# Alandroid/img-compression-mps

Measured on AMD Instinct MI355X. Metric: Mvoxels/s compress+reconstruct, 256^3 fp32, bond chi=64; SSIM vs ref, higher is better.
Workload: dtype f32

## Files before the change

### img-compression-mps_amd/_lib.py

```python
import ctypes as C
import os

_HERE = os.path.dirname(os.path.abspath(__file__))
LIB_PATH = os.path.join(_HERE, "libndmps_hip.so")

OK, EINVAL, EHIP, ENOCONV, EWORKSPACE, ETEAM = 0, -1, -2, -3, -4, -5

i64 = C.c_int64
p_i64 = C.POINTER(C.c_int64)
p_f64 = C.POINTER(C.c_double)
p_f32 = C.POINTER(C.c_float)
p_int = C.POINTER(C.c_int)
vp = C.c_void_p

SIGNATURES = {
    "ndmps_version": (C.c_int, []),
    "ndmps_last_error": (C.c_char_p, []),
    "ndmps_device_count": (C.c_int, []),
    "ndmps_streams_create": (C.c_int, [C.c_int, C.POINTER(vp), C.POINTER(C.c_int)]),
    "ndmps_streams_destroy": (C.c_int, [C.c_int, C.POINTER(vp)]),
    "ndmps_profile_enable": (C.c_int, [C.c_int]),
    "ndmps_profile_collect": (C.c_int, [C.c_int, p_f64, p_i64, p_i64]),
    "ndmps_plan_create": (C.c_int, [C.POINTER(vp), C.c_int, p_i64, C.c_int, p_i64]),
    "ndmps_plan_create_reversed": (C.c_int, [C.POINTER(vp), C.c_int, p_i64, C.c_int, p_i64]),
# ... 86 lines not shown
    "ndmps_syevj_batched_workspace_bytes": (i64, [i64, C.c_int]),
    "ndmps_syevj_batched_f64": (C.c_int, [C.c_int, vp, i64, p_i64, vp, i64, vp, i64, vp, i64, p_int, vp]),
    "ndmps_syevj_batched_tol_f64": (C.c_int, [C.c_int, vp, i64, p_i64, vp, i64, vp, i64, C.c_double, vp, i64,
                                              p_int, vp]),
    "ndmps_syevj_batched_values_f64": (C.c_int, [C.c_int, vp, i64, p_i64, vp, i64, vp, i64, C.c_double, vp, i64,
                                                 p_int, vp]),
    "ndmps_syevj_batched_vectors_f64": (C.c_int, [C.c_int, vp, i64, p_i64, vp, i64, vp, i64, p_i64, vp, i64, vp]),
    "ndmps_syevd_topk_max_n": (i64, []),
    "ndmps_syevd_topk_max_k": (i64, []),
    "ndmps_syevd_topk_max_k_wide": (i64, []),
    "ndmps_potrf_scratch_elems": (i64, [i64]),
    "ndmps_potrf_lower_f64": (C.c_int, [vp, i64, vp, C.POINTER(C.c_int), vp]),
    "ndmps_syevd_topk_workspace_bytes": (i64, [i64, C.c_int, i64]),
    "ndmps_syevd_topk_stamps_offset": (i64, [i64, C.c_int, i64]),
    "ndmps_syevd_topk_values_f64": (C.c_int, [C.c_int, vp, i64, p_i64, vp, i64, vp, i64, i64, vp, i64, vp]),
    "ndmps_syevd_topk_vectors_f64": (C.c_int, [C.c_int, p_i64, p_i64, i64, vp, i64, p_int, vp]),
    "ndmps_syevd_topk_vectors_auto_f64": (C.c_int, [C.c_int, p_i64, i64, C.c_double, vp, vp, i64, vp, vp, i64, vp]),
    "ndmps_syevd_topk_recover_f64": (C.c_int, [C.c_int, p_i64, i64, vp, i64, p_int, vp]),
    "ndmps_syevd_topk_set_team": (C.c_int, [C.c_int]),
    "ndmps_syevd_topk_set_streamed": (C.c_int, [C.c_int]),
    "ndmps_syevd_topk_team_fallbacks": (i64, []),
    "ndmps_syevd_topk_team_slots": (C.c_int, [i64]),
    "ndmps_syevd_topk_note_team_fallback": (C.c_int, []),
    "ndmps_debug_inject_team_abort": (C.c_int, [C.c_int]),
    "ndmps_debug_lane_sums_f64": (C.c_int, [vp, vp, vp]),
    "ndmps_tt_sweep_pads_cores": (C.c_int, [C.c_int, p_i64, i64]),
    "ndmps_tt_sweep_async_ints": (i64, [C.c_int, C.c_int]),
    "ndmps_tt_sweep_async_doubles": (i64, [C.c_int, C.c_int, p_i64, i64]),
    "ndmps_tt_sweep_batched_fused_begin_f32": (C.c_int, [C.c_int, C.POINTER(vp), C.c_int, p_i64, C.c_double, i64,
                                                         C.POINTER(vp), p_i64, p_i64, vp, vp, vp, vp, vp, i64,
                                                         vp, i64, vp, vp, vp]),
    "ndmps_tt_sweep_finish": (C.c_int, [C.c_int, C.c_int, p_i64, i64, vp, vp, p_i64, p_f64, p_i64]),
    "ndmps_tt_sweep_batched_workspace_bytes": (i64, [C.c_int, C.c_int, p_i64, i64]),
    "ndmps_tt_sweep_batched_f32": (C.c_int, [C.c_int, C.POINTER(vp), C.c_int, p_i64, C.c_double, i64,
                                             C.POINTER(vp), p_i64, p_i64, p_f64, p_i64, vp, i64, vp]),
    "ndmps_tt_layout": (C.c_int, [C.c_int, p_i64, i64, p_i64, p_i64, p_i64, p_i64]),
    "ndmps_tt_sweep_f32": (C.c_int, [vp, C.c_int, p_i64, C.c_double, i64, vp, p_i64, p_i64, p_f64,
                                     p_i64, vp, i64, vp]),
    "ndmps_compress_bond_workspace_bytes": (i64, [i64, i64, i64, i64, i64]),
    "ndmps_compress_bond_f32": (C.c_int, [vp, vp, i64, i64, i64, i64, i64, C.c_double, i64, vp, vp,
                                          p_i64, p_f64, vp, i64, vp]),
    "ndmps_chain_workspace_bytes": (i64, [C.c_int, p_i64, p_i64]),
    "ndmps_chain_contract_f32": (C.c_int, [C.c_int, p_i64, p_i64, C.POINTER(vp), vp, vp, i64, vp]),
    "ndmps_overlap_workspace_bytes": (i64, [C.c_int, p_i64, p_i64, p_i64]),
    "ndmps_overlap_f32": (C.c_int, [C.c_int, p_i64, p_i64, C.POINTER(vp), p_i64, C.POINTER(vp), p_f64,
                                    vp, i64, vp]),
# ... 96 lines not shown
```

### img-compression-mps_amd/csrc/eig_sym.inc

```
constexpr int kSymTiles = 17;

struct SymShared {
  double bc[4];
  RowVec rv[512];
  double red_a[4], red_b[4];
  double part[4][64];
  double rsum[kSymTiles * 32];
  int go;
};

template <int NB>
__device__ __forceinline__ void trd_sym_body(SymShared& sh, TrdDesc& d, const TrdWork& w, const int64_t b, const int wg) {
  constexpr int NR = 2, NT = kSymTiles;
  const int n = d.n;
  const int J = n - kTail;
  const int nblk = (n + 31) / 32;
  const int nphys = (nblk + 1) / 2;
  const int blkA = wg, blkB = nblk - 1 - wg;
  const int nA = nblk - blkA;
  const int nB = blkB != blkA ? NB : 0;
  const int j_last = min(J - 1, 32 * blkB + 30);
  const int lda = w.lda;
  const int tid = threadIdx.x, lane = tid & 63, wave = tid >> 6;
  double* A = w.A + b * w.n_max * lda;
  double* Vh = w.Vh + b * w.n_max * lda;
  double* ycol = w.y + b * 2 * lda;
  double* yrow = w.yrow + b * 2 * 8 * lda;
  double* xc = w.xc + b * 2 * lda;
  TeamSync* sync = w.sync + b;
  double (&bc)[4] = sh.bc;
  RowVec (&rv)[512] = sh.rv;
  double (&red_a)[4] = sh.red_a;
  double (&red_b)[4] = sh.red_b;
  double (&part)[4][64] = sh.part;
  double (&rsum)[kSymTiles * 32] = sh.rsum;
  int& go = sh.go;

  const int p = lane & 7, q = lane >> 3;
// ... 258 lines not shown
    const int r_lo = J >> 5;
#pragma unroll
    for (int r = 0; r < NR; ++r) {
      const int i = tid + 256 * r;
      if (i >= J && i < n) {
        double s = team_load(yc + i);
        const int bm = i >> 5;
        for (int ws = 0; ws < nphys; ++ws) {
          const int ra = ws, rb = nblk - 1 - ws;
          if ((ra >= r_lo && ra < bm) || (rb != ra && rb >= r_lo && rb < bm)) s += team_load(yr + (int64_t)ws * lda + i);
        }
        yc[i] = s;
      }
    }
  }
}

__global__ void __launch_bounds__(256, 2)
trd_sym_kernel(TrdDesc* __restrict__ desc, TrdWork w, int b0) {
  int wg, team;
  if (!team_place(w, wg, team)) return;
  const int64_t b = b0 + team;
  TrdDesc& d = desc[b];
  if (d.n - kTail <= 0 || wg >= ((d.n + 31) / 32 + 1) / 2) return;
  __shared__ SymShared sh;
  switch (wg) {
    case 0: trd_sym_body<1>(sh, d, w, b, wg); break;
    case 1: trd_sym_body<2>(sh, d, w, b, wg); break;
    case 2: trd_sym_body<3>(sh, d, w, b, wg); break;
    case 3: trd_sym_body<4>(sh, d, w, b, wg); break;
    case 4: trd_sym_body<5>(sh, d, w, b, wg); break;
    case 5: trd_sym_body<6>(sh, d, w, b, wg); break;
    case 6: trd_sym_body<7>(sh, d, w, b, wg); break;
    default: trd_sym_body<8>(sh, d, w, b, wg); break;
  }
}
```

### img-compression-mps_amd/csrc/eig_tridiag.hip

```cpp
#include <math.h>
#include <stdlib.h>
#include <string.h>

#include <algorithm>
#include <atomic>
#include <map>
#include <mutex>
#include <vector>

#include "common.h"
#include "lanes.h"

namespace {
__device__ __forceinline__ double load_if(const double* p, bool ok) {
  const double v = *p;
  return ok ? v : 0.0;
}
}

namespace {

typedef double f64x4 __attribute__((ext_vector_type(4)));

constexpr int kTail = 128;
constexpr int kTailLd = 132;
constexpr int kMaxK = 128;
constexpr int kMaxN = 4096;

struct TrdDesc {
  const double* G_in;
  double* V_out;
  double* w_out;
  int n;
  int k;
  int status;
  int pad;
};

struct __attribute__((aligned(16))) TeamRec {
  double v;
  unsigned long long tag;
};

struct TeamSync {
  unsigned long long count;
  int abort;
  int pad[317];
};
// ... 3 lines not shown
  double* Vh;
  double* y;
  double* xc;
  TeamRec* yr;
  TeamRec* xr;
  TeamSync* sync;
  double* tau;
  double* d;
  double* e;
  double* lam;
  double* mu;
  double* bound;
  double* Z;
  double* lu;
  unsigned char* piv;
  double* Tw;
  int64_t t_stride;
  double* yb;
  double* xb;
  double* band;
  double* qlog;
  int64_t q_stride;
  int tail_lower;
  int xcd_team, xcd_count;
  int xcd_pair;
  double* yrow;
  double* pv;
  double* pw;
  double* ypart;
  double* spart;
  double* ucol;
  double* napart;
  int pnl_blocks_max, pnl_tiles_max;
  long long* stamps;
  int n_max, lda, kp;
};

template <int STEPS>
__device__ __forceinline__ double fast_rsqrt(double x) {
  double y = __builtin_amdgcn_rsq(x);
#pragma unroll
  for (int i = 0; i < STEPS; ++i) y = y * fma(-0.5 * x * y, y, 1.5);
  return y;
}
template <int STEPS>
__device__ __forceinline__ double fast_rcp(double x) {
// ... 37 lines not shown
  const int n = d.n, lda = w.lda;
  const double* G = d.G_in;
  double* A = w.A + (int64_t)blockIdx.y * w.n_max * lda;
  const int64_t total = (int64_t)n * lda;
  for (int64_t e = (int64_t)blockIdx.x * 256 + threadIdx.x; e < total; e += (int64_t)gridDim.x * 256) {
    const int r = (int)(e / lda), c = (int)(e % lda);
    A[e] = c < n ? 0.5 * (G[(int64_t)r * n + c] + G[(int64_t)c * n + r]) : 0.0;
  }
}

struct __attribute__((aligned(16))) RowVec {
  double vp, wp, vj, pad;
};

template <int NR, int CW>
__global__ void __launch_bounds__(256)
trd_column_kernel(const TrdDesc* __restrict__ desc, TrdWork w, int j) {
  constexpr int LPR = CW / 2;
  constexpr int RPW = 64 / LPR;
  constexpr int RPI = 4 * RPW;
  constexpr int PRE = 512 / RPI;
  const TrdDesc& d = desc[blockIdx.y];
  const int n = d.n;
  if (j >= n - kTail) return;
  const int c0 = blockIdx.x * CW;
  if (c0 >= n || c0 + CW <= j + 1) return;
  const int lda = w.lda;
  const int tid = threadIdx.x, lane = tid & 63, wave = tid >> 6;
  const int64_t b = blockIdx.y;
  double* A = w.A + b * w.n_max * lda;
  double* Vh = w.Vh + b * w.n_max * lda;
  double* ybuf = w.y + b * 2 * lda;
  extern __shared__ __attribute__((aligned(16))) double lds[];
  RowVec* rv = reinterpret_cast<RowVec*>(lds);
  __shared__ double red_a[4], red_b[4];
  __shared__ double part[4][CW];

  const int q = lane / LPR, p = lane % LPR;
  const int c = c0 + 2 * p;
  const bool col_ok = c < lda;
  const int first = j + 1 + RPW * wave + q;
  double2 a[PRE];
#pragma unroll
  for (int u = 0; u < PRE; ++u) {
    const int i = first + RPI * u;
    a[u] = (i < n && col_ok) ? *reinterpret_cast<const double2*>(A + (int64_t)i * lda + c) : make_double2(0.0, 0.0);
  }
// ... 195 lines not shown
      const int blk = min(w.xcd_team, 32), pos = member % blk;
      member += blk - 1 - 2 * pos;
    }
  } else {
    const int r = w.xcd_count - full, l2 = L - full * w.xcd_team;
    member = l2 / r;
    team = full + l2 % r;
  }
  return true;
}

template <int NR, bool TAGGED, int CW = 32>
__global__ void __launch_bounds__(256, NR <= 4 ? 2 : 1)
trd_team_kernel(TrdDesc* __restrict__ desc, TrdWork w, int b0, unsigned epoch) {
  constexpr int MR = 256 * NR;
  constexpr int LPR = CW / 4;
  constexpr int RPW = 64 / LPR;
  constexpr int RPI = 4 * RPW;
  constexpr int NT = MR / RPI;
  int member, team;
  if (!team_place(w, member, team)) return;
  TrdDesc& d = desc[b0 + team];
  const int n = d.n;
  const int J = n - kTail;
  const int c0 = member * CW;
  if (J <= 0 || c0 >= n) return;
  const int nblk = (n + CW - 1) / CW;
  const int j_last = min(J - 1, c0 + CW - 2);
  const int lda = w.lda;
  const int tid = threadIdx.x, lane = tid & 63, wave = tid >> 6;
  const int64_t b = b0 + team;
  double* A = w.A + b * w.n_max * lda;
  double* Vh = w.Vh + b * w.n_max * lda;
  double* ybuf = w.y + b * 2 * lda;
  double* xc = w.xc + b * 2 * lda;
  TeamSync* sync = w.sync + b;
  TeamRec* yr = w.yr + b * 2 * lda;
  TeamRec* xr = w.xr + b * 2 * lda;
  const unsigned long long tag_base = (unsigned long long)epoch << 32;
  extern __shared__ __attribute__((aligned(32))) double team_dyn[];
  RowVec* rv = reinterpret_cast<RowVec*>(team_dyn);
  __shared__ double red_a[4], red_b[4];
  __shared__ double part[4][CW];
  __shared__ int go;

  const int q = lane % RPW, p = lane / RPW;
  const int c = c0 + 4 * p;
// ... 294 lines not shown
    __syncthreads();
    TEAM_STAMP(6)
    if (!go) return;
  }
#ifdef NDMPS_TEAM_STAMPS
  if (tid == 0 && member == nblk - 1)
    for (int q = 0; q < 8; ++q) w.stamps[b * 16 + q] = st[q];
#endif

  if (j_last == J - 1) {
    const int u0 = J / RPI;
#pragma unroll
    for (int u = 0; u < NT; ++u) {
      const int i = row0 + RPI * u;
      if (u >= u0 && i < n) {
        if (c < lda) *reinterpret_cast<double2*>(A + (int64_t)i * lda + c) = make_double2(a[u][0], a[u][1]);
        if (c + 2 < lda) *reinterpret_cast<double2*>(A + (int64_t)i * lda + c + 2) = make_double2(a[u][2], a[u][3]);
      }
    }
  }
}

__global__ void __launch_bounds__(512) trd_tail_kernel(const TrdDesc* __restrict__ desc, TrdWork w) {
  const TrdDesc& d = desc[blockIdx.y];
  const int n = d.n;
  const int J = max(n - kTail, 0), m = n - J;
  const int lda = w.lda;
  const int tid = threadIdx.x, lane = tid & 63, wave = tid >> 6;
  const int64_t b = blockIdx.y;
  const double* A = w.A + b * w.n_max * lda;
  double* Vh = w.Vh + b * w.n_max * lda;
  const double* ybuf = w.y + b * 2 * lda;
  double* dd = w.d + b * w.n_max;
  double* ee = w.e + b * w.n_max;
  double* tt = w.tau + b * w.n_max;
  extern __shared__ __attribute__((aligned(16))) double lds[];
  double* S = lds;
  RowVec* cv = reinterpret_cast<RowVec*>(lds + kTail * kTailLd);
  __shared__ double red_s[8], red_d[8];

  if (J >= 1) {
    const double* yprev = ybuf + ((J - 1) & 1) * lda;
    const double* vprev = Vh + (int64_t)(J - 1) * lda;
    const double taup = tt[J - 1];
    double dot = 0.0, vv = 0.0, y0 = 0.0;
    if (tid < m) {
      vv = vprev[J + tid];
      y0 = yprev[J + tid];
      dot = y0 * vv;
    }
    dot = wave_sum(dot);
    if (lane == 0) red_s[wave] = dot;
    __syncthreads();
    dot = 0.0;
#pragma unroll
    for (int x = 0; x < 8; ++x) dot += red_s[x];
    const double al = 0.5 * taup * taup * dot;
    if (tid < m) {
      cv[tid].vp = vv;
      cv[tid].wp = taup * y0 - al * vv;
    }
  } else if (tid < m) {
    cv[tid].vp = 0.0;
    cv[tid].wp = 0.0;
  }
  __syncthreads();
  for (int e = tid; e < m * m; e += 512) {
    const int r = e / m, c = e % m;
    const int gr = J + r, gc = J + c;
    const bool mirror = w.tail_lower && (gr >> 5) < (gc >> 5);
    const double av = mirror ? A[(int64_t)gc * lda + gr] : A[(int64_t)gr * lda + gc];
    S[r * kTailLd + c] = av - (cv[r].vp * cv[c].wp + cv[r].wp * cv[c].vp);
  }
  __syncthreads();
  if (tid < kTail) {
    cv[tid].vp = 0.0;
    cv[tid].wp = 0.0;
    cv[tid].vj = 0.0;
  }
  for (int e = tid; e < kTail * kTailLd; e += 512) {
    const int r = e / kTailLd, c = e % kTailLd;
    if (r >= m || c >= m) S[e] = 0.0;
  }
  __syncthreads();

  const int r = tid >> 2, t = tid & 3;
  for (int jj = 0; jj + 1 < m; ++jj) {
    const int j = J + jj;
    const double vpj = cv[jj].vp, wpj = cv[jj].wp;
    double a = 0.0, sigma = 0.0;
    if (tid < m && tid > jj) {
      a = S[jj * kTailLd + tid] - (vpj * cv[tid].wp + wpj * cv[tid].vp);
      if (tid > jj + 1) sigma = a * a;
    }
    sigma = wave_sum(sigma);
    if (lane == 0) red_s[wave] = sigma;
    const double alpha = S[jj * kTailLd + jj + 1] - (vpj * cv[jj + 1].wp + wpj * cv[jj + 1].vp);
    __syncthreads();
    sigma = 0.0;
#pragma unroll
    for (int x = 0; x < 8; ++x) sigma += red_s[x];
    double beta, tau, scale;
    householder(alpha, sigma, beta, tau, scale);
    const double vme = tid > jj + 1 ? a * scale : (tid == jj + 1 ? 1.0 : 0.0);
    if (tid < m) cv[tid].vj = vme;
    if (tid == 0) {
      dd[j] = S[jj * kTailLd + jj] - 2.0 * vpj * wpj;
      ee[j] = beta;
      tt[j] = tau;
    }
    __syncthreads();
    for (int i = tid; i < lda; i += 512) Vh[(int64_t)j * lda + i] = (i >= J && i < n) ? cv[i - J].vj : 0.0;
    double acc = 0.0;
    if (r < m && r > jj) {
      const RowVec me = cv[r];
      double* row = S + r * kTailLd;
      const int it0 = (jj + 1) >> 3;
#pragma unroll 4
      for (int it = it0; it < kTail / 8; ++it) {
        const int c = 2 * (t + 4 * it);
        double2 sv = *reinterpret_cast<double2*>(row + c);
        const RowVec c0v = cv[c], c1v = cv[c + 1];
        sv.x -= me.vp * c0v.wp + me.wp * c0v.vp;
        sv.y -= me.vp * c1v.wp + me.wp * c1v.vp;
        acc = fma(sv.x, c0v.vj, acc);
        acc = fma(sv.y, c1v.vj, acc);
        *reinterpret_cast<double2*>(row + c) = sv;
      }
    }
    acc = ndmps_lanes::sum_adjacent<4>(acc);
    const double vjr = r < kTail ? cv[r].vj : 0.0;
    double dot = (t == 0 && r < m && r > jj) ? acc * vjr : 0.0;
    dot = wave_sum(dot);
    if (lane == 0) red_d[wave] = dot;
    __syncthreads();
    dot = 0.0;
#pragma unroll
    for (int x = 0; x < 8; ++x) dot += red_d[x];
    const double al = 0.5 * tau * tau * dot;
    if (t == 0 && r < m) {
      const double yr = r > jj ? acc : 0.0;
      cv[r].wp = tau * yr - al * vjr;
      cv[r].vp = vjr;
    }
    __syncthreads();
  }
  if (tid == 0) {
    const int jj = m - 1;
    dd[n - 1] = S[jj * kTailLd + jj] - 2.0 * cv[jj].vp * cv[jj].wp;
    ee[n - 1] = 0.0;
    tt[n - 1] = 0.0;
  }
  for (int i = tid; i < lda; i += 512) Vh[(int64_t)(n - 1) * lda + i] = 0.0;
}

__global__ void __launch_bounds__(512) trd_tail_reg_kernel(const TrdDesc* __restrict__ desc, TrdWork w) {
  const TrdDesc& d = desc[blockIdx.y];
  const int n = d.n;
  const int J = max(n - kTail, 0), m = n - J;
  const int lda = w.lda;
  const int tid = threadIdx.x, lane = tid & 63, wave = tid >> 6;
  const int64_t b = blockIdx.y;
  const double* A = w.A + b * w.n_max * lda;
  double* Vh = w.Vh + b * w.n_max * lda;
  const double* ybuf = w.y + b * 2 * lda;
  double* dd = w.d + b * w.n_max;
  double* ee = w.e + b * w.n_max;
  double* tt = w.tau + b * w.n_max;
  __shared__ RowVec cv[kTail];
  __shared__ double xrow[kTail];
  __shared__ double yv[kTail];
  __shared__ double red_s[8];
// ... 1215 lines not shown
  w.mu = (double*)(base + l.off_mu);
  w.bound = (double*)(base + l.off_bound);
  w.Z = (double*)(base + l.off_z);
  w.lu = (double*)(base + l.off_lu);
  w.piv = (unsigned char*)(base + l.off_piv);
  w.stamps = (long long*)(base + l.off_stamps);
  w.Tw = (double*)(base + l.off_tw);
  w.t_stride = l.t_stride;
  w.yb = (double*)(base + l.off_yb);
  w.xb = (double*)(base + l.off_xb);
  w.band = (double*)(base + l.off_band);
  w.qlog = (double*)(base + l.off_qlog);
  w.q_stride = l.q_stride;
  w.yrow = (double*)(base + l.off_yrow);
  w.pv = (double*)(base + l.off_pv);
  w.pw = (double*)(base + l.off_pw);
  w.ypart = (double*)(base + l.off_ypart);
  w.spart = (double*)(base + l.off_spart);
  w.ucol = (double*)(base + l.off_ucol);
  w.napart = (double*)(base + l.off_napart);
  w.pnl_blocks_max = (int)l.pnl_blocks;
  w.pnl_tiles_max = (int)l.pnl_tiles;
  w.tail_lower = 0;
  w.xcd_team = w.xcd_count = w.xcd_pair = 0;
  w.n_max = (int)l.n_max;
  w.lda = (int)l.lda;
  w.kp = (int)l.kp;
  return w;
}

constexpr int kInvitLdsMax = kMaxK * (kMaxK + 1) * 8;
constexpr size_t kTailLds = ((size_t)kTail * kTailLd + 4 * kTail) * sizeof(double);

thread_local int g_team_off = 0;
thread_local int g_team_streamed = 0;
std::atomic<long long> g_team_fallbacks{0};
std::atomic<int> g_inject_abort{0};


int trd_opt_in() {
  static std::mutex mu;
  static bool done[64] = {};
  int dev = 0;
  NDMPS_CHECK_HIP(hipGetDevice(&dev));
  std::lock_guard<std::mutex> lock(mu);
  if (dev < 0 || dev >= 64 || done[dev]) return NDMPS_OK;
  NDMPS_CHECK_HIP(hipFuncSetAttribute(reinterpret_cast<const void*>(&trd_tail_kernel),
                                      hipFuncAttributeMaxDynamicSharedMemorySize, (int)kTailLds));
  NDMPS_CHECK_HIP(hipFuncSetAttribute(reinterpret_cast<const void*>(&trd_team_kernel<8, true, 8>),
                                      hipFuncAttributeMaxDynamicSharedMemorySize, 2048 * (int)sizeof(RowVec)));
  NDMPS_CHECK_HIP(hipFuncSetAttribute(reinterpret_cast<const void*>(&trd_column_kernel<16, 32>),
                                      hipFuncAttributeMaxDynamicSharedMemorySize, kMaxN * (int)sizeof(RowVec)));
  NDMPS_CHECK_HIP(hipFuncSetAttribute(reinterpret_cast<const void*>(&trd_column_kernel<16, 8>),
                                      hipFuncAttributeMaxDynamicSharedMemorySize, kMaxN * (int)sizeof(RowVec)));
  NDMPS_CHECK_HIP(hipFuncSetAttribute(reinterpret_cast<const void*>(&trd_invit_kernel),
                                      hipFuncAttributeMaxDynamicSharedMemorySize, kInvitLdsMax));
  NDMPS_CHECK_HIP(hipFuncSetAttribute(reinterpret_cast<const void*>(&trd_ortho_kernel<true>),
                                      hipFuncAttributeMaxDynamicSharedMemorySize, kInvitLdsMax));
  NDMPS_CHECK_HIP(hipFuncSetAttribute(reinterpret_cast<const void*>(&trd_ortho_kernel<false>),
                                      hipFuncAttributeMaxDynamicSharedMemorySize, kInvitLdsMax));
  NDMPS_CHECK_HIP(hipFuncSetAttribute(reinterpret_cast<const void*>(&wide_chol_diag_kernel),
                                      hipFuncAttributeMaxDynamicSharedMemorySize, 2 * kWB * kWLd * (int)sizeof(double)));
  NDMPS_CHECK_HIP(hipFuncSetAttribute(reinterpret_cast<const void*>(&trd_ortho_blocks_kernel),
                                      hipFuncAttributeMaxDynamicSharedMemorySize, 3 * 64 * 65 * 8));
  NDMPS_CHECK_HIP(hipFuncSetAttribute(reinterpret_cast<const void*>(&trd_back2_kernel<2>),
                                      hipFuncAttributeMaxDynamicSharedMemorySize, 512 * 32 * 8));
  NDMPS_CHECK_HIP(hipFuncSetAttribute(reinterpret_cast<const void*>(&trd_back2_kernel<4>),
                                      hipFuncAttributeMaxDynamicSharedMemorySize, 512 * 32 * 8));
  done[dev] = true;
  return NDMPS_OK;
}
// ... 214 lines not shown
      for (int b0 = 0; b0 < batch; b0 += per_launch) {
        const unsigned epoch = g_team_epoch.fetch_add(1);
        const int count = std::min(per_launch, batch - b0);
        TrdWork wl = w;
        dim3 grid((unsigned)team_size, (unsigned)count);
        if (xcd_placed) {
          wl.xcd_team = team_size;
          wl.xcd_count = count;
          const bool pairable = 32 % team_size == 0 || team_size % 32 == 0;
          wl.xcd_pair = sym || !pairable ? 0 : getenv("NDMPS_TRD_PAIR") ? atoi(getenv("NDMPS_TRD_PAIR")) : 1;
          grid = dim3((unsigned)(team_size * count));
        }
        if (sym) hipLaunchKernelGGL(trd_sym_kernel, grid, dim3(256), 0, s, desc, wl, b0);
        else if (narrow_team) hipLaunchKernelGGL((trd_team_kernel<2, true, 8>), grid, dim3(256), 512 * sizeof(RowVec), s, desc, wl, b0, epoch);
        else hipLaunchKernelGGL((trd_team_kernel<2, false>), grid, dim3(256), 512 * sizeof(RowVec), s, desc, wl, b0, epoch);
      }
    }, (int64_t)std::min(per_launch, batch) * team_size <= slots / 2));
  return NDMPS_OK;
}

int trd_reduce_and_values(int batch, const int64_t* h_n, int64_t n_max, int64_t k_max, const TrdLayout& l, const TrdWork& w_in,
                          TrdDesc* desc, hipStream_t s) {
  TrdWork w = w_in;
  const unsigned B = (unsigned)batch;
  const int load_grid = (int)std::min<int64_t>(ndmps::ceil_div(n_max * l.lda, 256), 512);
  hipLaunchKernelGGL(trd_load_kernel, dim3(load_grid, B), dim3(256), 0, s, desc, w);
  const bool narrow = (int64_t)batch * ndmps::ceil_div(n_max, 8) <= 2 * ndmps::kNumCU && !getenv("NDMPS_TRD_WIDE");
  const int W = (int)ndmps::ceil_div(n_max, narrow ? 8 : 32);
  const size_t col_lds = (size_t)n_max * sizeof(RowVec);
  void (*column)(const TrdDesc*, TrdWork, int);
  if (narrow)
    column = n_max <= 512    ? trd_column_kernel<2, 8>
             : n_max <= 1024 ? trd_column_kernel<4, 8>
             : n_max <= 2048 ? trd_column_kernel<8, 8>
                             : trd_column_kernel<16, 8>;
  else
    column = n_max <= 512    ? trd_column_kernel<2, 32>
             : n_max <= 1024 ? trd_column_kernel<4, 32>
             : n_max <= 2048 ? trd_column_kernel<8, 32>
                             : trd_column_kernel<16, 32>;
  const int bw = band_width_for(n_max);
  route_store(w_in.A, bw);
  const bool team = !bw && n_max <= 512 && n_max > kTail && !getenv("NDMPS_TRD_NO_TEAM") && !g_team_off;
  if (bw) {
    int slots = 0;
    NDMPS_TRY(team_slots(slots));
    const int team_size = (int)ndmps::ceil_div(n_max, 32);
    const int per_launch = std::max(1, slots / team_size);
    int inject = g_inject_abort.load();
    while (inject > 0 && !g_inject_abort.compare_exchange_weak(inject, inject - 1)) {
    }
    void* span = ndmps::span_begin(s);
    if (inject > 0) {
      hipLaunchKernelGGL(trd_inject_abort_kernel, dim3((batch + 63) / 64), dim3(64), 0, s, desc, batch);
    } else {
      NDMPS_TRY(team_launch(s, [&]() {
        for (int b0 = 0; b0 < batch; b0 += per_launch) {
          const dim3 grid((unsigned)team_size, (unsigned)std::min(per_launch, batch - b0));
          if (bw == 2) hipLaunchKernelGGL(trd_band_kernel<2>, grid, dim3(256), 0, s, desc, w, b0);
          else hipLaunchKernelGGL(trd_band_kernel<4>, grid, dim3(256), 0, s, desc, w, b0);
        }
      }));
    }
    int64_t bytes = 0;
    for (int b = 0; b < batch; ++b) bytes += 2 * 8 * h_n[b] * h_n[b];
    ndmps::span_end(span, s, ndmps::kSpanTridiagTeam, 1, bytes);
// ... 17 lines not shown
  bool big_team = false;
  if (team_on && n_max > 512 && n_max <= std::min<int64_t>(team_max, 2048)) NDMPS_TRY(team_fits(n_max, big_team));
  int hybrid = 0;
  if (team_on && !big_team && n_max > 512 && n_max % 2 == 0 && !getenv("NDMPS_TRD_NO_HYBRID")) {
    bool uniform = true;
    for (int b = 0; b < batch && uniform; ++b) uniform = h_n[b] == n_max;
    for (int h = 2048; h >= 512 && uniform && !hybrid; h /= 2) {
      bool fits = false;
      if (h > team_max || n_max - h < kPnlTB) continue;
      NDMPS_TRY(team_fits(h, fits));
      if (fits) hybrid = h;
    }
  }
  void* span = ndmps::span_begin(s);
  int64_t span_bytes = 0;
  if (team || big_team) {
    NDMPS_TRY(trd_team_reduce(batch, n_max, desc, w, s));
    for (int b = 0; b < batch; ++b) span_bytes += 2 * 8 * h_n[b] * h_n[b];
    ndmps::span_end(span, s, ndmps::kSpanTridiagTeam, 1, span_bytes);
  } else if (n_max >= panel_min_order(hybrid != 0) && !getenv("NDMPS_TRD_NO_PANEL")) {
    NDMPS_CHECK_HIP(hipMemsetAsync(w.Vh, 0, (size_t)batch * n_max * l.lda * 8, s));
    NDMPS_CHECK_HIP(hipMemsetAsync(w.pv, 0, (size_t)batch * n_max * kPnlNB * 8, s));
    NDMPS_CHECK_HIP(hipMemsetAsync(w.pw, 0, (size_t)batch * n_max * kPnlNB * 8, s));
    const int tail_cols = hybrid ? hybrid : kTail;
    w.tail_lower = hybrid ? 0 : 1;
    const int J_max = (int)n_max - tail_cols;
    std::vector<char> ends((size_t)J_max + 1, 0);
    for (int b = 0; b < batch; ++b) ends[(size_t)std::max<int64_t>(h_n[b] - tail_cols, 0)] = 1;
    const int nbm = (int)l.pnl_blocks;
    auto tiles = [&](int first_col) {
      const int nblk = nbm - first_col / kPnlTB;
      return (unsigned)(nblk * (nblk + 1) / 2);
    };
    std::vector<PnlLaunch> seq;
    seq.reserve((size_t)2 * J_max + J_max / kPnlNB + 4);
    for (int j = 0; j <= J_max; ++j) {
      seq.push_back({0, (unsigned)(nbm - j / kPnlTB), j});
      if (j >= 1 && (j % kPnlNB == 0 || ends[(size_t)j])) seq.push_back({1, tiles(j), j});
      if (j < J_max) seq.push_back({2, tiles(j + 1), j});
      if (span)
        for (int b = 0; b < batch; ++b)
          if (j < h_n[b] - tail_cols) span_bytes += 4 * (h_n[b] - j - 1) * (h_n[b] - j - 1);
    }
    NDMPS_TRY(pnl_run(seq, batch, h_n, n_max, tail_cols, desc, w, s));
    if (hybrid) {
      const int64_t J0 = n_max - hybrid;
      TrdDesc* sub = (TrdDesc*)((char*)w_in.A - l.off_a + l.off_desc2);
      hipLaunchKernelGGL(pnl_mirror_kernel, dim3(256, B), dim3(256), 0, s, w, (int)n_max, hybrid);
      hipLaunchKernelGGL(pnl_subdesc_kernel, dim3((batch + 63) / 64), dim3(64), 0, s, (const TrdDesc*)desc, sub, batch, hybrid);
      TrdWork v = w;
      v.A = w.A + J0 * l.lda + J0;
      v.Vh = w.Vh + J0 * l.lda + J0;
      v.y = w.y + J0;
      v.tau = w.tau + J0;
      v.d = w.d + J0;
      v.e = w.e + J0;
      NDMPS_TRY(trd_team_reduce(batch, hybrid, sub, v, s));
      hipLaunchKernelGGL(pnl_substatus_kernel, dim3((batch + 63) / 64), dim3(64), 0, s, desc, (const TrdDesc*)sub, batch);
      w.tail_lower = 0;
    } else {
      NDMPS_CHECK_HIP(hipMemsetAsync(w.y, 0, (size_t)batch * 2 * l.lda * 8, s));
    }
    ndmps::span_end(span, s, ndmps::kSpanTridiagPanel, (int64_t)seq.size(), span_bytes);
  } else {
    for (int j = 0; j < n_max - kTail; ++j) {
      hipLaunchKernelGGL(column, dim3(W, B), dim3(256), col_lds, s, desc, w, j);
      if (span)
        for (int b = 0; b < batch; ++b)
          if (j < h_n[b] - kTail) span_bytes += 2 * 8 * (h_n[b] - j - 1) * (h_n[b] - j - 1);
    }
    ndmps::span_end(span, s, ndmps::kSpanTridiagColumns, std::max<int64_t>(n_max - kTail, 0), span_bytes);
  }
  const char* tail_env = getenv("NDMPS_TRD_TAIL");
  const bool tail_regs = tail_env ? !strcmp(tail_env, "regs") : batch < 16;
  void* tail_span = ndmps::span_begin(s);
  if (tail_regs) hipLaunchKernelGGL(trd_tail_reg_kernel, dim3(1, B), dim3(512), 0, s, desc, w);
  else hipLaunchKernelGGL(trd_tail_kernel, dim3(1, B), dim3(512), kTailLds, s, desc, w);
  const int kk = (int)std::min(k_max, n_max);
  hipLaunchKernelGGL(trd_bisect_kernel, dim3(ndmps::ceil_div(kk, 4), B), dim3(256),
                     (size_t)ndmps::round_up(n_max, 16) * 16, s, desc, w, kk);
  ndmps::span_end(tail_span, s, ndmps::kSpanTridiagTail, 2, 0);
  NDMPS_LAUNCH_CHECK();
  return NDMPS_OK;
}

}

extern "C" int64_t ndmps_potrf_scratch_elems(int64_t n) {
  const int64_t kw = ndmps::round_up(std::max<int64_t>(n, 1), kWB);
  return kw * kw + 64;
}
extern "C" int ndmps_potrf_lower_f64(double* d_S, int64_t n, double* d_scratch, int* h_status, ndmps_stream_t stream) {
  NDMPS_REQUIRE(d_S && d_scratch && h_status && n >= 1 && n <= 32768, "bad Cholesky argument");
  NDMPS_TRY(trd_opt_in());
  hipStream_t s = (hipStream_t)stream;
  const int k = (int)n, kw = (int)ndmps::round_up(n, kWB), nblk = kw / kWB;
  double* linv = d_scratch;
  TrdDesc* d_flag = reinterpret_cast<TrdDesc*>(d_scratch + (int64_t)kw * kw);
  NDMPS_CHECK_HIP(hipMemsetAsync(d_flag, 0, sizeof(TrdDesc), s));
  for (int pb = 0; pb < nblk; ++pb) {
// ... 298 lines not shown
  g_team_fallbacks.fetch_add(1);
  hipLaunchKernelGGL(trd_clear_status_kernel, dim3((batch + 63) / 64), dim3(64), 0, s, desc, batch, w.sync);
  g_team_off += 1;
  const int rc = trd_reduce_and_values(batch, h_n, n_max, k_max, l, w, desc, s);
  g_team_off -= 1;
  return rc;
}
extern "C" int ndmps_syevd_topk_set_team(int enabled) {
  const int was = g_team_off ? 0 : 1;
  g_team_off = enabled ? 0 : 1;
  return was;
}
extern "C" int ndmps_syevd_topk_set_streamed(int streamed) {
  const int was = g_team_streamed;
  g_team_streamed = streamed ? 1 : 0;
  return was;
}
extern "C" int64_t ndmps_syevd_topk_team_fallbacks(void) { return g_team_fallbacks.load(); }
extern "C" int ndmps_syevd_topk_team_slots(int64_t order) {
  int slots = 0;
  if (trd_opt_in() != NDMPS_OK || team_slots(slots, order <= 512 ? 2 : order <= 1024 ? 4 : 8) != NDMPS_OK) return 0;
  return slots;
}
extern "C" int ndmps_syevd_topk_note_team_fallback(void) {
  g_team_fallbacks.fetch_add(1);
  return NDMPS_OK;
}
namespace {
__global__ void lane_sums_kernel(const double* __restrict__ in, double* __restrict__ out) {
  const int l = threadIdx.x;
  const double v = in[l];
  using namespace ndmps_lanes;
  out[0 * 64 + l] = sum_adjacent<2>(v);
  out[1 * 64 + l] = sum_adjacent<4>(v);
  out[2 * 64 + l] = sum_adjacent<8>(v);
  out[3 * 64 + l] = sum_adjacent<16>(v);
  out[4 * 64 + l] = sum_adjacent<32>(v);
  out[5 * 64 + l] = sum_adjacent<64>(v);
  out[6 * 64 + l] = sum_strided<1>(v);
  out[7 * 64 + l] = sum_strided<2>(v);
  out[8 * 64 + l] = sum_strided<4>(v);
  out[9 * 64 + l] = sum_strided<8>(v);
  out[10 * 64 + l] = sum_strided<16>(v);
  out[11 * 64 + l] = sum_strided<32>(v);
}
}
// ... 13 lines not shown
```

### include/ndmps_hip.h

```cpp
#ifndef NDMPS_HIP_H
#define NDMPS_HIP_H

#include <stdint.h>

#ifdef __cplusplus
extern "C" {
#endif

#define NDMPS_OK 0
#define NDMPS_EINVAL (-1)
#define NDMPS_EHIP (-2)
#define NDMPS_ENOCONV (-3)
#define NDMPS_EWORKSPACE (-4)
#define NDMPS_ETEAM (-5)

typedef void* ndmps_stream_t;
typedef struct ndmps_plan ndmps_plan_t;

int ndmps_version(void);
const char* ndmps_last_error(void);
int ndmps_device_count(void);

int ndmps_streams_create(int n, void** h_streams, int* n_independent);
int ndmps_streams_destroy(int n, void* const* h_streams);
// ... 113 lines not shown
                                    double* d_V, int64_t stride_V, double* d_w, int64_t stride_w,
                                    const int64_t* h_k, void* d_ws, int64_t ws_bytes,
                                    ndmps_stream_t stream);

int64_t ndmps_syevd_topk_max_n(void);
int64_t ndmps_syevd_topk_max_k(void);
int64_t ndmps_syevd_topk_max_k_wide(void);
int64_t ndmps_syevd_topk_workspace_bytes(int64_t n_max, int batch, int64_t k_max);
int64_t ndmps_syevd_topk_stamps_offset(int64_t n_max, int batch, int64_t k_max);
int64_t ndmps_potrf_scratch_elems(int64_t n);
int ndmps_potrf_lower_f64(double* d_S, int64_t n, double* d_scratch, int* h_status, ndmps_stream_t stream);
int ndmps_syevd_topk_values_f64(int batch, const double* d_G, int64_t stride_G, const int64_t* h_n,
                                double* d_V, int64_t stride_V, double* d_w, int64_t stride_w,
                                int64_t k_max, void* d_ws, int64_t ws_bytes, ndmps_stream_t stream);
int ndmps_syevd_topk_vectors_f64(int batch, const int64_t* h_n, const int64_t* h_k, int64_t k_max,
                                 void* d_ws, int64_t ws_bytes, int* h_status, ndmps_stream_t stream);
int ndmps_syevd_topk_recover_f64(int batch, const int64_t* h_n, int64_t k_max, void* d_ws, int64_t ws_bytes,
                                 int* h_recovered, ndmps_stream_t stream);
int ndmps_syevd_topk_set_team(int enabled);
int ndmps_syevd_topk_set_streamed(int streamed);
int64_t ndmps_syevd_topk_team_fallbacks(void);
int ndmps_syevd_topk_team_slots(int64_t order);
int ndmps_syevd_topk_note_team_fallback(void);
int ndmps_debug_inject_team_abort(int launches);
int ndmps_debug_lane_sums_f64(const double* d_in, double* d_out, ndmps_stream_t stream);
int ndmps_syevd_topk_vectors_auto_f64(int batch, const int64_t* h_n, int64_t k_cap, double cutoff,
                                      int* d_ranks, double* d_spectra, int64_t spectra_stride,
                                      int* d_status, void* d_ws, int64_t ws_bytes, ndmps_stream_t stream);

int ndmps_tt_layout(int L, const int64_t* h_dims, int64_t max_bond, int64_t* h_max_bonds,
                    int64_t* h_core_offsets, int64_t* h_spec_offsets,
                    int64_t* h_workspace_bytes);
int ndmps_tt_sweep_f32(float* d_dense, int L, const int64_t* h_dims, double cutoff,
                       int64_t max_bond, float* d_cores, const int64_t* h_core_offsets,
                       int64_t* h_bonds_out, double* h_spectra, const int64_t* h_spec_offsets,
                       void* d_ws, int64_t ws_bytes, ndmps_stream_t stream);

int ndmps_tt_sweep_pads_cores(int L, const int64_t* h_dims, int64_t max_bond);
int64_t ndmps_tt_sweep_async_ints(int batch, int L);
int64_t ndmps_tt_sweep_async_doubles(int batch, int L, const int64_t* h_dims, int64_t max_bond);
int ndmps_tt_sweep_batched_fused_begin_f32(int batch, const float* const* h_volume, int L, const int64_t* h_dims,
                                           double cutoff, int64_t max_bond, float* const* h_cores,
                                           const int64_t* h_core_offsets, int64_t* h_bonds_scratch,
                                           const int64_t* d_row_off, const int64_t* d_row_off_sorted,
                                           const int32_t* d_row_order, const int64_t* d_col_off,
                                           const int32_t* d_col_perm, int64_t n_cols, void* d_ws, int64_t ws_bytes,
// ... 172 lines not shown
```

Before: 42380.

## Store LDS tridiagonal tail as packed lower-triangular 32x32 blocks and enlarge it

Measured after the change: 41700. 1.6% lower.

```diff
diff --git a/img-compression-mps_amd/_lib.py b/img-compression-mps_amd/_lib.py
--- a/img-compression-mps_amd/_lib.py
+++ b/img-compression-mps_amd/_lib.py
@@ -132,6 +132,10 @@
     "ndmps_syevd_topk_team_fallbacks": (i64, []),
     "ndmps_syevd_topk_team_slots": (C.c_int, [i64]),
     "ndmps_syevd_topk_note_team_fallback": (C.c_int, []),
+    "ndmps_syevd_topk_handover_column": (i64, [i64, C.c_int]),
+    "ndmps_syevd_topk_tail_order": (i64, []),
+    "ndmps_syevd_topk_tail_elems": (i64, []),
+    "ndmps_syevd_topk_tail_slot": (i64, [i64, i64]),
     "ndmps_debug_inject_team_abort": (C.c_int, [C.c_int]),
     "ndmps_debug_lane_sums_f64": (C.c_int, [vp, vp, vp]),
     "ndmps_tt_sweep_pads_cores": (C.c_int, [C.c_int, p_i64, i64]),
diff --git a/img-compression-mps_amd/csrc/eig_sym.inc b/img-compression-mps_amd/csrc/eig_sym.inc
--- a/img-compression-mps_amd/csrc/eig_sym.inc
+++ b/img-compression-mps_amd/csrc/eig_sym.inc
@@ -13,7 +13,7 @@
 __device__ __forceinline__ void trd_sym_body(SymShared& sh, TrdDesc& d, const TrdWork& w, const int64_t b, const int wg) {
   constexpr int NR = 2, NT = kSymTiles;
   const int n = d.n;
-  const int J = n - kTail;
+  const int J = n - w.tail_cols;
   const int nblk = (n + 31) / 32;
   const int nphys = (nblk + 1) / 2;
   const int blkA = wg, blkB = nblk - 1 - wg;
@@ -318,7 +318,7 @@
   if (!team_place(w, wg, team)) return;
   const int64_t b = b0 + team;
   TrdDesc& d = desc[b];
-  if (d.n - kTail <= 0 || wg >= ((d.n + 31) / 32 + 1) / 2) return;
+  if (d.n - w.tail_cols <= 0 || wg >= ((d.n + 31) / 32 + 1) / 2) return;
   __shared__ SymShared sh;
   switch (wg) {
     case 0: trd_sym_body<1>(sh, d, w, b, wg); break;
diff --git a/img-compression-mps_amd/csrc/eig_tridiag.hip b/img-compression-mps_amd/csrc/eig_tridiag.hip
--- a/img-compression-mps_amd/csrc/eig_tridiag.hip
+++ b/img-compression-mps_amd/csrc/eig_tridiag.hip
@@ -23,7 +23,23 @@
 typedef double f64x4 __attribute__((ext_vector_type(4)));
 
 constexpr int kTail = 128;
-constexpr int kTailLd = 132;
+constexpr int kTailLds = 160;
+constexpr int kTailBlk = 32;
+constexpr int kTailBlkLd = 33;
+constexpr int kTailNb = kTailLds / kTailBlk;
+constexpr int kTailBlocks = kTailNb * (kTailNb + 1) / 2;
+constexpr int kTailBlkElems = kTailBlk * kTailBlkLd;
+constexpr int kTailElems = kTailBlocks * kTailBlkElems;
+static_assert(kTailLds % kTailBlk == 0, "whole block-columns are handed over");
+static_assert((size_t)kTailElems * 8 + (size_t)kTailLds * 32 + 3968 + 1120 + 512 * 32 <= 160 * 1024,
+              "LDS tail + one resident workgroup exceed a CU's LDS");
+
+__host__ __device__ __forceinline__ int tail_slot(int r, int c) {
+  const int br = r / kTailBlk, bc = c / kTailBlk;
+  const int hi = br >= bc ? r : c, lo = br >= bc ? c : r;
+  const int bh = hi / kTailBlk, bl = lo / kTailBlk;
+  return (bh * (bh + 1) / 2 + bl) * kTailBlkElems + (hi % kTailBlk) * kTailBlkLd + lo % kTailBlk;
+}
 constexpr int kMaxK = 128;
 constexpr int kMaxN = 4096;
 
@@ -73,6 +89,7 @@
   double* qlog;
   int64_t q_stride;
   int tail_lower;
+  int tail_cols;
   int xcd_team, xcd_count;
   int xcd_pair;
   double* yrow;
@@ -156,7 +173,7 @@
   constexpr int PRE = 512 / RPI;
   const TrdDesc& d = desc[blockIdx.y];
   const int n = d.n;
-  if (j >= n - kTail) return;
+  if (j >= n - w.tail_cols) return;
   const int c0 = blockIdx.x * CW;
   if (c0 >= n || c0 + CW <= j + 1) return;
   const int lda = w.lda;
@@ -398,7 +415,7 @@
   if (!team_place(w, member, team)) return;
   TrdDesc& d = desc[b0 + team];
   const int n = d.n;
-  const int J = n - kTail;
+  const int J = n - w.tail_cols;
   const int c0 = member * CW;
   if (J <= 0 || c0 >= n) return;
   const int nblk = (n + CW - 1) / CW;
@@ -739,9 +756,10 @@
 }
 
 __global__ void __launch_bounds__(512) trd_tail_kernel(const TrdDesc* __restrict__ desc, TrdWork w) {
+  static_assert(kTailNb == 5, "the block decode of the fill loop");
   const TrdDesc& d = desc[blockIdx.y];
   const int n = d.n;
-  const int J = max(n - kTail, 0), m = n - J;
+  const int J = max(n - w.tail_cols, 0), m = n - J;
   const int lda = w.lda;
   const int tid = threadIdx.x, lane = tid & 63, wave = tid >> 6;
   const int64_t b = blockIdx.y;
@@ -753,8 +771,9 @@
   double* tt = w.tau + b * w.n_max;
   extern __shared__ __attribute__((aligned(16))) double lds[];
   double* S = lds;
-  RowVec* cv = reinterpret_cast<RowVec*>(lds + kTail * kTailLd);
+  RowVec* cv = reinterpret_cast<RowVec*>(lds + kTailElems);
   __shared__ double red_s[8], red_d[8];
+  __shared__ double part[3][kTailLds];
 
   if (J >= 1) {
     const double* yprev = ybuf + ((J - 1) & 1) * lda;
@@ -782,37 +801,43 @@
     cv[tid].wp = 0.0;
   }
   __syncthreads();
-  for (int e = tid; e < m * m; e += 512) {
-    const int r = e / m, c = e % m;
-    const int gr = J + r, gc = J + c;
-    const bool mirror = w.tail_lower && (gr >> 5) < (gc >> 5);
-    const double av = mirror ? A[(int64_t)gc * lda + gr] : A[(int64_t)gr * lda + gc];
-    S[r * kTailLd + c] = av - (cv[r].vp * cv[c].wp + cv[r].wp * cv[c].vp);
+  const int nb = (m + kTailBlk - 1) / kTailBlk;
+  for (int e = tid; e < kTailBlocks * kTailBlk * kTailBlk; e += 512) {
+    const int blk = e >> 10, ri = (e >> 5) & 31, ci = e & 31;
+    const int bi = blk < 1 ? 0 : blk < 3 ? 1 : blk < 6 ? 2 : blk < 10 ? 3 : 4, bj = blk - bi * (bi + 1) / 2;
+    if (bi >= nb) break;
+    const int r = kTailBlk * bi + ri, c = kTailBlk * bj + ci;
+    double v = 0.0;
+    if (r < m && c < m) {
+      const int gr = J + r, gc = J + c;
+      const bool mirror = w.tail_lower && (gr >> 5) < (gc >> 5);
+      const double av = mirror ? A[(int64_t)gc * lda + gr] : A[(int64_t)gr * lda + gc];
+      v = av - (cv[r].vp * cv[c].wp + cv[r].wp * cv[c].vp);
+    }
+    S[blk * kTailBlkElems + ri * kTailBlkLd + ci] = v;
   }
   __syncthreads();
-  if (tid < kTail) {
+  if (tid < kTailLds) {
     cv[tid].vp = 0.0;
     cv[tid].wp = 0.0;
     cv[tid].vj = 0.0;
   }
-  for (int e = tid; e < kTail * kTailLd; e += 512) {
-    const int r = e / kTailLd, c = e % kTailLd;
-    if (r >= m || c >= m) S[e] = 0.0;
-  }
   __syncthreads();
 
-  const int r = tid >> 2, t = tid & 3;
+  const int uc = tid & 31, ur = tid >> 5;
+  const int t = tid / kTailLds, r = tid - t * kTailLds;
+  const int rb = r / kTailBlk, ri = r % kTailBlk;
   for (int jj = 0; jj + 1 < m; ++jj) {
     const int j = J + jj;
     const double vpj = cv[jj].vp, wpj = cv[jj].wp;
     double a = 0.0, sigma = 0.0;
     if (tid < m && tid > jj) {
-      a = S[jj * kTailLd + tid] - (vpj * cv[tid].wp + wpj * cv[tid].vp);
+      a = S[tail_slot(tid, jj)] - (vpj * cv[tid].wp + wpj * cv[tid].vp);
       if (tid > jj + 1) sigma = a * a;
     }
     sigma = wave_sum(sigma);
     if (lane == 0) red_s[wave] = sigma;
-    const double alpha = S[jj * kTailLd + jj + 1] - (vpj * cv[jj + 1].wp + wpj * cv[jj + 1].vp);
+    const double alpha = S[tail_slot(jj + 1, jj)] - (vpj * cv[jj + 1].wp + wpj * cv[jj + 1].vp);
     __syncthreads();
     sigma = 0.0;
 #pragma unroll
@@ -822,32 +847,43 @@
     const double vme = tid > jj + 1 ? a * scale : (tid == jj + 1 ? 1.0 : 0.0);
     if (tid < m) cv[tid].vj = vme;
     if (tid == 0) {
-      dd[j] = S[jj * kTailLd + jj] - 2.0 * vpj * wpj;
+      dd[j] = S[tail_slot(jj, jj)] - 2.0 * vpj * wpj;
       ee[j] = beta;
       tt[j] = tau;
     }
     __syncthreads();
     for (int i = tid; i < lda; i += 512) Vh[(int64_t)j * lda + i] = (i >= J && i < n) ? cv[i - J].vj : 0.0;
-    double acc = 0.0;
-    if (r < m && r > jj) {
-      const RowVec me = cv[r];
-      double* row = S + r * kTailLd;
-      const int it0 = (jj + 1) >> 3;
-#pragma unroll 4
-      for (int it = it0; it < kTail / 8; ++it) {
-        const int c = 2 * (t + 4 * it);
-        double2 sv = *reinterpret_cast<double2*>(row + c);
-        const RowVec c0v = cv[c], c1v = cv[c + 1];
-        sv.x -= me.vp * c0v.wp + me.wp * c0v.vp;
-        sv.y -= me.vp * c1v.wp + me.wp * c1v.vp;
-        acc = fma(sv.x, c0v.vj, acc);
-        acc = fma(sv.y, c1v.vj, acc);
-        *reinterpret_cast<double2*>(row + c) = sv;
-      }
-    }
-    acc = ndmps_lanes::sum_adjacent<4>(acc);
-    const double vjr = r < kTail ? cv[r].vj : 0.0;
-    double dot = (t == 0 && r < m && r > jj) ? acc * vjr : 0.0;
+    const int b_lo = (jj + 1) / kTailBlk;
+    for (int bi = b_lo; bi < nb; ++bi) {
+      const RowVec r0 = cv[kTailBlk * bi + ur], r1 = cv[kTailBlk * bi + ur + 16];
+      for (int bj = b_lo; bj <= bi; ++bj) {
+        const RowVec cc = cv[kTailBlk * bj + uc];
+        double* p = S + (bi * (bi + 1) / 2 + bj) * kTailBlkElems + ur * kTailBlkLd + uc;
+        p[0] -= r0.vp * cc.wp + r0.wp * cc.vp;
+        p[16 * kTailBlkLd] -= r1.vp * cc.wp + r1.wp * cc.vp;
+      }
+    }
+    __syncthreads();
+    const bool live = t < 3 && r < m && r > jj;
+    double acc0 = 0.0, acc1 = 0.0;
+    if (live) {
+      for (int bj = b_lo; bj < nb; ++bj) {
+        const bool direct = bj <= rb;
+        const int st = direct ? 1 : kTailBlkLd;
+        const double* p = S + (direct ? (rb * (rb + 1) / 2 + bj) * kTailBlkElems + ri * kTailBlkLd
+                                      : (bj * (bj + 1) / 2 + rb) * kTailBlkElems + ri) + t * st;
+        const RowVec* cr = cv + kTailBlk * bj + t;
+#pragma unroll
+        for (int k = 0; k < 10; k += 2) {
+          acc0 = fma(p[3 * k * st], cr[3 * k].vj, acc0);
+          acc1 = fma(p[(3 * k + 3) * st], cr[3 * k + 3].vj, acc1);
+        }
+        if (t < 2) acc0 = fma(p[30 * st], cr[30].vj, acc0);
+      }
+    }
+    const double acc = acc0 + acc1;
+    if (t < 3) part[t][r] = live ? acc : 0.0;
+    double dot = live ? acc * cv[r].vj : 0.0;
     dot = wave_sum(dot);
     if (lane == 0) red_d[wave] = dot;
     __syncthreads();
@@ -855,16 +891,16 @@
 #pragma unroll
     for (int x = 0; x < 8; ++x) dot += red_d[x];
     const double al = 0.5 * tau * tau * dot;
-    if (t == 0 && r < m) {
-      const double yr = r > jj ? acc : 0.0;
-      cv[r].wp = tau * yr - al * vjr;
-      cv[r].vp = vjr;
+    if (tid < m) {
+      const double yr = (part[0][tid] + part[1][tid]) + part[2][tid];
+      cv[tid].wp = tau * yr - al * vme;
+      cv[tid].vp = vme;
     }
     __syncthreads();
   }
   if (tid == 0) {
     const int jj = m - 1;
-    dd[n - 1] = S[jj * kTailLd + jj] - 2.0 * cv[jj].vp * cv[jj].wp;
+    dd[n - 1] = S[tail_slot(jj, jj)] - 2.0 * cv[jj].vp * cv[jj].wp;
     ee[n - 1] = 0.0;
     tt[n - 1] = 0.0;
   }
@@ -2126,6 +2162,7 @@
   w.pnl_blocks_max = (int)l.pnl_blocks;
   w.pnl_tiles_max = (int)l.pnl_tiles;
   w.tail_lower = 0;
+  w.tail_cols = kTail;
   w.xcd_team = w.xcd_count = w.xcd_pair = 0;
   w.n_max = (int)l.n_max;
   w.lda = (int)l.lda;
@@ -2134,7 +2171,13 @@
 }
 
 constexpr int kInvitLdsMax = kMaxK * (kMaxK + 1) * 8;
-constexpr size_t kTailLds = ((size_t)kTail * kTailLd + 4 * kTail) * sizeof(double);
+constexpr size_t kTailLdsBytes = (size_t)kTailElems * sizeof(double) + kTailLds * sizeof(RowVec);
+
+bool tail_in_registers(int batch) {
+  const char* tail_env = getenv("NDMPS_TRD_TAIL");
+  return tail_env ? !strcmp(tail_env, "regs") : batch < 16;
+}
+int tail_cols_for(int batch) { return tail_in_registers(batch) ? kTail : kTailLds; }
 
 thread_local int g_team_off = 0;
 thread_local int g_team_streamed = 0;
@@ -2150,7 +2193,7 @@
   std::lock_guard<std::mutex> lock(mu);
   if (dev < 0 || dev >= 64 || done[dev]) return NDMPS_OK;
   NDMPS_CHECK_HIP(hipFuncSetAttribute(reinterpret_cast<const void*>(&trd_tail_kernel),
-                                      hipFuncAttributeMaxDynamicSharedMemorySize, (int)kTailLds));
+                                      hipFuncAttributeMaxDynamicSharedMemorySize, (int)kTailLdsBytes));
   NDMPS_CHECK_HIP(hipFuncSetAttribute(reinterpret_cast<const void*>(&trd_team_kernel<8, true, 8>),
                                       hipFuncAttributeMaxDynamicSharedMemorySize, 2048 * (int)sizeof(RowVec)));
   NDMPS_CHECK_HIP(hipFuncSetAttribute(reinterpret_cast<const void*>(&trd_column_kernel<16, 32>),
@@ -2411,6 +2454,9 @@
 int trd_reduce_and_values(int batch, const int64_t* h_n, int64_t n_max, int64_t k_max, const TrdLayout& l, const TrdWork& w_in,
                           TrdDesc* desc, hipStream_t s) {
   TrdWork w = w_in;
+  const bool tail_regs = tail_in_registers(batch);
+  const int tail_cols = tail_cols_for(batch);
+  w.tail_cols = tail_cols;
   const unsigned B = (unsigned)batch;
   const int load_grid = (int)std::min<int64_t>(ndmps::ceil_div(n_max * l.lda, 256), 512);
   hipLaunchKernelGGL(trd_load_kernel, dim3(load_grid, B), dim3(256), 0, s, desc, w);
@@ -2430,7 +2476,7 @@
                              : trd_column_kernel<16, 32>;
   const int bw = band_width_for(n_max);
   route_store(w_in.A, bw);
-  const bool team = !bw && n_max <= 512 && n_max > kTail && !getenv("NDMPS_TRD_NO_TEAM") && !g_team_off;
+  const bool team = !bw && n_max <= 512 && n_max > tail_cols && !getenv("NDMPS_TRD_NO_TEAM") && !g_team_off;
   if (bw) {
     int slots = 0;
     NDMPS_TRY(team_slots(slots));
@@ -2494,11 +2540,11 @@
     NDMPS_CHECK_HIP(hipMemsetAsync(w.Vh, 0, (size_t)batch * n_max * l.lda * 8, s));
     NDMPS_CHECK_HIP(hipMemsetAsync(w.pv, 0, (size_t)batch * n_max * kPnlNB * 8, s));
     NDMPS_CHECK_HIP(hipMemsetAsync(w.pw, 0, (size_t)batch * n_max * kPnlNB * 8, s));
-    const int tail_cols = hybrid ? hybrid : kTail;
+    const int pnl_cols = hybrid ? hybrid : tail_cols;
     w.tail_lower = hybrid ? 0 : 1;
-    const int J_max = (int)n_max - tail_cols;
+    const int J_max = (int)n_max - pnl_cols;
     std::vector<char> ends((size_t)J_max + 1, 0);
-    for (int b = 0; b < batch; ++b) ends[(size_t)std::max<int64_t>(h_n[b] - tail_cols, 0)] = 1;
+    for (int b = 0; b < batch; ++b) ends[(size_t)std::max<int64_t>(h_n[b] - pnl_cols, 0)] = 1;
     const int nbm = (int)l.pnl_blocks;
     auto tiles = [&](int first_col) {
       const int nblk = nbm - first_col / kPnlTB;
@@ -2512,9 +2558,9 @@
       if (j < J_max) seq.push_back({2, tiles(j + 1), j});
       if (span)
         for (int b = 0; b < batch; ++b)
-          if (j < h_n[b] - tail_cols) span_bytes += 4 * (h_n[b] - j - 1) * (h_n[b] - j - 1);
-    }
-    NDMPS_TRY(pnl_run(seq, batch, h_n, n_max, tail_cols, desc, w, s));
+          if (j < h_n[b] - pnl_cols) span_bytes += 4 * (h_n[b] - j - 1) * (h_n[b] - j - 1);
+    }
+    NDMPS_TRY(pnl_run(seq, batch, h_n, n_max, pnl_cols, desc, w, s));
     if (hybrid) {
       const int64_t J0 = n_max - hybrid;
       TrdDesc* sub = (TrdDesc*)((char*)w_in.A - l.off_a + l.off_desc2);
@@ -2535,19 +2581,17 @@
     }
     ndmps::span_end(span, s, ndmps::kSpanTridiagPanel, (int64_t)seq.size(), span_bytes);
   } else {
-    for (int j = 0; j < n_max - kTail; ++j) {
+    for (int j = 0; j < n_max - tail_cols; ++j) {
       hipLaunchKernelGGL(column, dim3(W, B), dim3(256), col_lds, s, desc, w, j);
       if (span)
         for (int b = 0; b < batch; ++b)
-          if (j < h_n[b] - kTail) span_bytes += 2 * 8 * (h_n[b] - j - 1) * (h_n[b] - j - 1);
-    }
-    ndmps::span_end(span, s, ndmps::kSpanTridiagColumns, std::max<int64_t>(n_max - kTail, 0), span_bytes);
-  }
-  const char* tail_env = getenv("NDMPS_TRD_TAIL");
-  const bool tail_regs = tail_env ? !strcmp(tail_env, "regs") : batch < 16;
+          if (j < h_n[b] - tail_cols) span_bytes += 2 * 8 * (h_n[b] - j - 1) * (h_n[b] - j - 1);
+    }
+    ndmps::span_end(span, s, ndmps::kSpanTridiagColumns, std::max<int64_t>(n_max - tail_cols, 0), span_bytes);
+  }
   void* tail_span = ndmps::span_begin(s);
   if (tail_regs) hipLaunchKernelGGL(trd_tail_reg_kernel, dim3(1, B), dim3(512), 0, s, desc, w);
-  else hipLaunchKernelGGL(trd_tail_kernel, dim3(1, B), dim3(512), kTailLds, s, desc, w);
+  else hipLaunchKernelGGL(trd_tail_kernel, dim3(1, B), dim3(512), kTailLdsBytes, s, desc, w);
   const int kk = (int)std::min(k_max, n_max);
   hipLaunchKernelGGL(trd_bisect_kernel, dim3(ndmps::ceil_div(kk, 4), B), dim3(256),
                      (size_t)ndmps::round_up(n_max, 16) * 16, s, desc, w, kk);
@@ -2892,6 +2936,16 @@
   if (trd_opt_in() != NDMPS_OK || team_slots(slots, order <= 512 ? 2 : order <= 1024 ? 4 : 8) != NDMPS_OK) return 0;
   return slots;
 }
+extern "C" int64_t ndmps_syevd_topk_handover_column(int64_t n, int batch) {
+  if (n <= 0 || n > kMaxN || batch <= 0) return -1;
+  return std::max<int64_t>(n - tail_cols_for(batch), 0);
+}
+extern "C" int64_t ndmps_syevd_topk_tail_order(void) { return kTailLds; }
+extern "C" int64_t ndmps_syevd_topk_tail_elems(void) { return kTailElems; }
+extern "C" int64_t ndmps_syevd_topk_tail_slot(int64_t r, int64_t c) {
+  if (r < 0 || c < 0 || r >= kTailLds || c >= kTailLds) return -1;
+  return tail_slot((int)r, (int)c);
+}
 extern "C" int ndmps_syevd_topk_note_team_fallback(void) {
   g_team_fallbacks.fetch_add(1);
   return NDMPS_OK;
diff --git a/include/ndmps_hip.h b/include/ndmps_hip.h
--- a/include/ndmps_hip.h
+++ b/include/ndmps_hip.h
@@ -159,6 +159,10 @@
 int64_t ndmps_syevd_topk_team_fallbacks(void);
 int ndmps_syevd_topk_team_slots(int64_t order);
 int ndmps_syevd_topk_note_team_fallback(void);
+int64_t ndmps_syevd_topk_handover_column(int64_t n, int batch);
+int64_t ndmps_syevd_topk_tail_order(void);
+int64_t ndmps_syevd_topk_tail_elems(void);
+int64_t ndmps_syevd_topk_tail_slot(int64_t r, int64_t c);
 int ndmps_debug_inject_team_abort(int launches);
 int ndmps_debug_lane_sums_f64(const double* d_in, double* d_out, ndmps_stream_t stream);
 int ndmps_syevd_topk_vectors_auto_f64(int batch, const int64_t* h_n, int64_t k_cap, double cutoff,
```
